# domkirke/acids_transforms

Measured on AMD Instinct MI355X. Metric: spectrogram frames/sec (fwd+invert), n_fft=1024 hop=256, higher is better.
Workload: dtype f32; 1 GPU; configs[1]: batch=1024 clips/GPU x 4 s mono 44.1 kHz, STFT fwd + Magnitude(mel=128, log1p, unipolar) [one fused kernel] + ISTFT invert, fp32; n_fft=1024, hop=256, frames_per_clip=690, clips_per_gpu=1024

## Files before the change

acids_transforms_amd/_lib.py:

```python
import ctypes
import os
import subprocess

import torch

_HERE = os.path.dirname(os.path.abspath(__file__))
_SO = os.environ.get("ACIDS_HIP_LIB") or os.path.join(_HERE, "libacids_hip.so")

ABI_VERSION = 4
AT_OK, AT_EINVAL, AT_EUNSUPPORTED, AT_ENOTINIT, AT_EWORKSPACE, AT_ELAUNCH = 0, -1, -2, -3, -4, -5

c_f = ctypes.c_void_p
c_i64 = ctypes.c_int64
c_int = ctypes.c_int
c_sz = ctypes.c_size_t
c_flt = ctypes.c_float

_SIGNATURES = {
    "at_abi_version": [],
    "at_error_string": [c_int],
    "at_init": [c_int],
    "at_set_variant": [c_int, c_int],
    "at_get_variant": [c_int],
    "at_stft_forward": [c_f, c_i64, c_i64, c_i64, c_i64, c_int, c_int, c_int, c_f, c_f, c_f, c_f],
    "at_stft_mel_forward": [c_f, c_i64, c_i64, c_i64, c_i64, c_int, c_int, c_f, c_f, c_f, c_f, c_int, c_int,
                            c_f, c_int, c_int, c_f, c_f, c_flt, c_f, c_f, c_f, c_int, c_f],
    "at_stft_polar_forward": [c_f, c_i64, c_i64, c_i64, c_i64, c_int, c_int, c_f, c_f, c_f, c_f, c_int, c_int, c_f,
                              c_int, c_f, c_f, c_flt, c_f, c_f, c_f, c_f],
    "at_istft_envelope_table": [c_f, c_int, c_int, c_f, c_f],
    "at_istft_workspace_bytes": [c_i64, c_i64, c_int, c_int],
    "at_istft": [c_f, c_f, c_f, c_i64, c_i64, c_int, c_int, c_f, c_f, c_f, c_f, c_sz, c_f],
    "at_irfft_frames": [c_f, c_f, c_f, c_i64, c_int, c_f, c_f, c_f],
    "at_irfft_frames_streams": [c_f, c_f, c_f, c_i64, c_i64, c_int, c_f, c_f, c_f],
    "at_angle": [c_f, c_i64, c_f, c_f],
    "at_phase_scan": [c_f, c_f, c_i64, c_i64, c_i64, c_int, c_int, c_f, c_f, c_f, c_f, c_f],
    "at_phase_integrate": [c_f, c_i64, c_i64, c_i64, c_int, c_int, c_f, c_f, c_f, c_f],
    "at_polar_to_complex": [c_f, c_f, c_i64, c_f, c_f],
    "at_phase_scan_strided": [c_f, c_f, c_i64, c_i64, c_i64, c_int, c_int, c_f, c_f, c_f, c_f, c_i64, c_f],
    "at_polarif_forward": [c_f, c_i64, c_i64, c_i64, c_int, c_f, c_f, c_f, c_f, c_f, c_f, c_f, c_i64, c_int, c_f, c_f, c_flt,
                           c_f, c_f],
    "at_phase_integrate_polar": [c_f, c_i64, c_i64, c_i64, c_i64, c_int, c_f, c_f, c_f, c_f, c_f],
    "at_cartesian_pack": [c_f, c_i64, c_int, c_f, c_f, c_f, c_f, c_f, c_f],
    "at_cartesian_unpack": [c_f, c_i64, c_int, c_f, c_f, c_f, c_f, c_f, c_f],
    "at_resample_sinc": [c_f, c_i64, c_i64, c_int, c_int, c_int, c_f, c_i64, c_f, c_f],
    "at_sinebank_workspace_bytes": [c_i64, c_int, c_i64, c_int],
    "at_sinebank_offline": [c_f, c_i64, c_i64, c_int, c_f, c_f, c_f, c_i64, c_int, c_f, c_f, c_f, c_f, c_f, c_sz, c_f],
    "at_sinebank_realtime": [c_f, c_i64, c_int, c_int, c_int, c_f, c_f, c_f, c_f, c_f, c_f],
    "at_mel_project": [c_f, c_int, c_i64, c_i64, c_int, c_f, c_int, c_int, c_int, c_int, c_f, c_f, c_flt, c_f, c_i64,
                       c_i64, c_f],
    "at_mel_project_banded": [c_f, c_int, c_i64, c_i64, c_int, c_f, c_f, c_f, c_int, c_int, c_f, c_int, c_int, c_f, c_f,
                              c_flt, c_f, c_i64, c_i64, c_f, c_i64, c_f, c_f, c_f, c_f],
    "at_mel_bf16_bank_bytes": [c_int, c_int],
    "at_mel_bf16_pack_bank": [c_f, c_int, c_int, c_int, c_f, c_f],
    "at_mel_project_bf16": [c_f, c_int, c_i64, c_i64, c_int, c_f, c_int, c_int, c_f, c_f, c_flt, c_f, c_i64, c_f],
    "at_project_small": [c_f, c_i64, c_int, c_f, c_int, c_f, c_f, c_f, c_i64, c_f],
    "at_mag_pointwise": [c_f, c_int, c_i64, c_int, c_int, c_f, c_f, c_flt, c_f, c_f],
    "at_stats_workspace_bytes": [],
    "at_stats": [c_f, c_int, c_i64, c_int, c_flt, c_f, c_f, c_sz, c_f],
    "at_affine": [c_f, c_i64, c_f, c_f, c_int, c_f, c_f],
    "at_pghi_gradients": [c_f, c_i64, c_int, c_int, c_flt, c_int, c_int, c_flt, c_f, c_f, c_f, c_f],
    "at_pghi_offline_workspace_bytes": [c_i64, c_int, c_int],
    "at_pghi_offline": [c_f, c_i64, c_int, c_int, c_flt, c_int, c_int, c_flt, c_flt, c_f, c_f, c_sz, c_f, c_f, c_f],
    "at_pghi_integrate": [c_f, c_f, c_f, c_i64, c_int, c_int, c_flt, c_flt, c_f, c_f, c_sz, c_f, c_f, c_f],
    "at_pghi_rt_workspace_bytes": [c_int, c_int, c_int],
    "at_pghi_realtime": [c_f, c_f, c_f, c_f, c_int, c_int, c_int, c_flt, c_int, c_int, c_flt, c_flt, c_f, c_f, c_f,
                         c_f, c_sz, c_f],
    "at_pghi_realtime_seeded": [c_f, c_f, c_f, c_f, c_int, c_int, c_int, c_flt, c_int, c_int, c_flt, c_flt, c_f, c_f, c_sz,
                                c_f],
    "at_rt_update_buffers": [c_f, c_f, c_int, c_int, c_int, c_f, c_f, c_f, c_f],
    "at_griffinlim_update": [c_f, c_f, c_f, c_flt, c_i64, c_f, c_f],
    "at_istft_griffinlim": [c_f, c_f, c_f, c_flt, c_i64, c_i64, c_int, c_int, c_f, c_f, c_f, c_f],
    "at_scale_complex": [c_f, c_f, c_i64, c_f, c_f],
    "at_oadd_forward": [c_f, c_f, c_int, c_i64, c_int, c_i64, c_f, c_f, c_f],
    "at_oadd_invert": [c_f, c_f, c_int, c_int, c_int, c_int, c_int, c_f, c_f, c_f, c_f],
    "at_oadd_push": [c_f, c_int, c_i64, c_int, c_i64, c_f, c_f],
    "at_mulaw_encode": [c_f, c_i64, c_int, c_f, c_f],
    "at_mulaw_decode": [c_f, c_f, c_i64, c_int, c_f, c_f],
    "at_onehot": [c_f, c_i64, c_int, c_i64, c_f, c_f],
    "at_argmax_last": [c_f, c_f, c_i64, c_int, c_f, c_f],
    "at_stft_backward_workspace_bytes": [c_i64, c_i64, c_int, c_int],
    "at_stft_backward": [c_f, c_i64, c_i64, c_i64, c_int, c_int, c_f, c_f, c_f, c_sz, c_f],
    "at_istft_backward_workspace_bytes": [c_i64, c_i64, c_int, c_int],
    "at_istft_backward": [c_f, c_i64, c_i64, c_int, c_int, c_f, c_f, c_f, c_f, c_f, c_sz, c_f],
    "at_magnitude_backward": [c_f, c_int, c_i64, c_int, c_f, c_int, c_int, c_f, c_f, c_f, c_f, c_int, c_f, c_f, c_f, c_f,
                              c_int, c_int, c_f, c_flt, c_f, c_f, c_f],
    "at_mfcc_backward": [c_f, c_i64, c_i64, c_int, c_f, c_int, c_int, c_int, c_f, c_f, c_f, c_f, c_int, c_f, c_f, c_f, c_f,
                         c_int, c_f, c_f, c_f, c_f],
}
_RESTYPES = {"at_error_string": ctypes.c_char_p, "at_istft_workspace_bytes": c_sz, "at_stats_workspace_bytes": c_sz,
             "at_pghi_offline_workspace_bytes": c_sz, "at_mel_bf16_bank_bytes": c_sz, "at_pghi_rt_workspace_bytes": c_sz,
             "at_sinebank_workspace_bytes": c_sz, "at_stft_backward_workspace_bytes": c_sz,
             "at_istft_backward_workspace_bytes": c_sz}


class AcidsHipError(RuntimeError):
    pass


def build(verbose=False):
    cmd = ["make", "-C", os.path.join(_HERE, "csrc"), "-j4"]
    if not verbose:
        cmd.append("-s")
    subprocess.check_call(cmd)
    return _SO
# ... 110 lines not shown
```

acids_transforms_amd/csrc/capi.hip:

```cpp
#include <hip/hip_runtime.h>
#include <math.h>
#include <stdint.h>
#include <vector>

#include "../../include/acids_hip.h"
#include "autograd.h"
#include "band_bank.h"
#include "fft512.h"

#include <atomic>
#include "variants.h"
namespace at_hip {
int launch_stft1024_fwd(const float*, long long, long long, long long, long long, int, int, const float*,
                        const float2*, float2*, float*, hipStream_t);
int launch_stft1024_h256_fwd(const float*, long long, long long, long long, long long, const float*, const float2*,
                             float2*, float*, const BandBank*, float*, const float*, const float*, float, int, int, int,
                             hipStream_t, const PolarOut* polar = nullptr, int hop = 256);
int launch_istft1024_ola(const float2*, const float*, const float*, long long, long long, int, const float*,
                         const float*, const float2*, float*, hipStream_t, const float2* gl_tprev = nullptr,
                         float gl_mom = 0.f);
int launch_irfft1024_frames(const float2*, const float*, const float*, long long, const float*, const float2*,
                            float*, hipStream_t);
int launch_rfft_generic(const float*, long long, long long, long long, long long, int, int, int, const float*,
                        float2*, float*, hipStream_t);
// ... 15 lines not shown
                         const float*, const float2*, const float2*, float*, hipStream_t);
int launch_stft4096_fwd(const float*, long long, long long, long long, long long, int, int, const float*, const float2*,
                        const float2*, float2*, float*, hipStream_t);
int launch_istft4096_ola(const float2*, const float*, const float*, long long, long long, int, const float*, const float*,
                         const float2*, const float2*, float*, hipStream_t);
int launch_irfft4096_frames(const float2*, const float*, const float*, long long, const float*, const float2*,
                            const float2*, float*, hipStream_t);
int launch_stft_small_fwd(int, const float*, long long, long long, long long, long long, int, int, const float*, const float2*,
                          const float2*, float2*, float*, hipStream_t);
int launch_irfft_small_frames(int, const float2*, const float*, const float*, long long, long long, const float*,
                              const float2*, const float2*, float*, hipStream_t);
int launch_stft512_fwd(const float*, long long, long long, long long, long long, int, int, const float*, const float2*,
                       const float2*, float2*, float*, hipStream_t);
int launch_irfft512_frames(const float2*, const float*, const float*, long long, long long, const float*, const float2*,
                           const float2*, float*, hipStream_t);
int launch_istft512_ola(const float2*, const float*, const float*, long long, long long, int, const float*, const float*,
                        const float2*, const float2*, float*, hipStream_t);

constexpr int kMaxDevices = 16;
static float2* g_twiddles[kMaxDevices] = {nullptr};
static float2* g_tw2048[kMaxDevices] = {nullptr};

static const float2* twiddles_for_current_device() {
  int dev = 0;
  if (hipGetDevice(&dev) != hipSuccess || dev < 0 || dev >= kMaxDevices) return nullptr;
  return g_twiddles[dev];
}

static const float2* tw2048_for_current_device() {
  int dev = 0;
  if (hipGetDevice(&dev) != hipSuccess || dev < 0 || dev >= kMaxDevices) return nullptr;
  return g_tw2048[dev];
}

static bool is_pow2(int n) { return n > 0 && (n & (n - 1)) == 0; }
static bool fft_size_ok(int n) { return n >= 2 && n <= 16384 && (!(n & 1) || n < 8192); }
static bool fft_mixed(int n) { return !is_pow2(n) || n < 8; }

__global__ void envelope_table_kernel(const float* w, int n_fft, int hop, int R, float* env) {
  int i = blockIdx.x * blockDim.x + threadIdx.x;
  if (i >= (1 << R) * hop) return;
  int mask = i / hop, r = i - mask * hop;
  float s = 0.f;
  for (int q = 0; q < R; ++q)
    if (mask & (1 << q)) {
      int o = hop * (R - 1 - q) + r;
      if (o < n_fft) s += w[o] * w[o];
    }
  env[i] = s;
}
static std::atomic<int> g_variants[kVarCount];
int variant(int which) { return g_variants[which].load(std::memory_order_relaxed); }
}

using namespace at_hip;

extern "C" {

int at_abi_version(void) { return 4; }

int at_set_variant(int which, int value) {
  if (which < 0 || which >= kVarCount || value < 0 || value > (which >= kVarFirstPlan ? 65535 : 4)) return AT_EINVAL;
  g_variants[which].store(value, std::memory_order_relaxed);
  return AT_OK;
}

int at_get_variant(int which) {
  if (which < 0 || which >= kVarCount) return AT_EINVAL;
  return g_variants[which].load(std::memory_order_relaxed);
}

const char* at_error_string(int code) {
  switch (code) {
    case AT_OK: return "ok";
    case AT_EINVAL: return "invalid argument";
    case AT_EUNSUPPORTED: return "unsupported configuration";
    case AT_ENOTINIT: return "at_init() not called for this device";
    case AT_EWORKSPACE: return "workspace too small";
    case AT_ELAUNCH: return "HIP launch/runtime error";
    default: return "unknown error";
  }
}

int at_init(int device) {
  if (device < 0 || device >= kMaxDevices) return AT_EINVAL;
  if (g_twiddles[device]) return AT_OK;
  int prev = 0;
  if (hipGetDevice(&prev) != hipSuccess) return AT_ELAUNCH;
  if (hipSetDevice(device) != hipSuccess) return AT_ELAUNCH;
  std::vector<float2> tab(kTwiddleCount);
  const double two_pi = 6.283185307179586476925286766559;
  for (int k = 1; k < 8; ++k)
    for (int l = 0; l < 64; ++l) {
      double a1 = -two_pi * (double)(l * k) / 512.0;
      tab[(k - 1) * 64 + l] = make_float2((float)cos(a1), (float)sin(a1));
      double a2 = -two_pi * (double)((l & 7) * k) / 64.0;
      tab[(7 + k - 1) * 64 + l] = make_float2((float)cos(a2), (float)sin(a2));
    }
  for (int m = 0; m < 8; ++m)
    for (int l = 0; l < 64; ++l) {
      double a = -two_pi * (double)(l + 64 * m) / 1024.0;
      tab[(14 + m) * 64 + l] = make_float2((float)cos(a), (float)sin(a));
    }
  float2* d = nullptr;
  int rc = AT_OK;
  if (hipMalloc((void**)&d, sizeof(float2) * (kTwiddleCount + kTileCtrSlots)) != hipSuccess) rc = AT_ELAUNCH;
  if (rc == AT_OK && hipMemcpy(d, tab.data(), sizeof(float2) * kTwiddleCount, hipMemcpyHostToDevice) != hipSuccess)
    rc = AT_ELAUNCH;
  if (rc == AT_OK && hipMemset(d + kTwiddleCount, 0, sizeof(float2) * kTileCtrSlots) != hipSuccess) rc = AT_ELAUNCH;
  float2* d2 = nullptr;
  if (rc == AT_OK) {
    std::vector<float2> t2(1024 + 256 + 384 + 448 + 2048 + 1536);
    for (int k = 0; k < 2048; ++k) {
      const double a = -two_pi * (double)k / 4096.0;
      t2[2112 + k] = make_float2((float)cos(a), (float)sin(a));
    }
    for (int r = 1; r < 4; ++r)
      for (int k = 0; k < 512; ++k) {
        const double a = -two_pi * (double)(r * k) / 2048.0;
        t2[4160 + (r - 1) * 512 + k] = make_float2((float)cos(a), (float)sin(a));
      }
    for (int r = 1; r < 4; ++r)
      for (int k = 0; k < 128; ++k) {
        const double a = -two_pi * (double)(r * k) / 512.0;
        t2[1280 + (r - 1) * 128 + k] = make_float2((float)cos(a), (float)sin(a));
      }
    for (int r = 1; r < 8; ++r)
      for (int k = 0; k < 64; ++k) {
        const double a = -two_pi * (double)(r * k) / 512.0;
        t2[1664 + (r - 1) * 64 + k] = make_float2((float)cos(a), (float)sin(a));
      }
    for (int k = 0; k < 1024; ++k) {
      const double a = -two_pi * (double)k / 2048.0;
      t2[k] = make_float2((float)cos(a), (float)sin(a));
    }
    for (int k = 0; k < 256; ++k) {
      const double a = -two_pi * (double)k / 512.0;
      t2[1024 + k] = make_float2((float)cos(a), (float)sin(a));
    }
    if (hipMalloc((void**)&d2, sizeof(float2) * t2.size()) != hipSuccess) rc = AT_ELAUNCH;
    if (rc == AT_OK && hipMemcpy(d2, t2.data(), sizeof(float2) * t2.size(), hipMemcpyHostToDevice) != hipSuccess)
      rc = AT_ELAUNCH;
  }
  if (rc == AT_OK) {
    g_tw2048[device] = d2;
    g_twiddles[device] = d;
  }
  (void)hipSetDevice(prev);
  return rc;
}

int at_stft_forward(const float* x, int64_t B, int64_t L, int64_t clip_stride, int64_t T, int n_fft, int hop,
                    int center, const float* window, float* out_complex, float* phase, void* stream) {
  if (B < 0 || T < 0 || L < 0 || hop <= 0 || n_fft <= 0) return AT_EINVAL;
  if (B * T == 0) return AT_OK;
  if (!x || !window || !out_complex) return AT_EINVAL;
  if (!fft_size_ok(n_fft)) return AT_EUNSUPPORTED;
  if (center && L <= n_fft / 2) return AT_EINVAL;
  hipStream_t s = (hipStream_t)stream;
  if (n_fft == 1024 && (((uintptr_t)window) & 7) == 0) {
    const float2* tw = twiddles_for_current_device();
    if (!tw) return AT_ENOTINIT;
    if ((hop == 256 || hop == 128 || hop == 512) && center && (clip_stride & 1) == 0)
      return launch_stft1024_h256_fwd(x, B, L, clip_stride, T, window, tw, (float2*)out_complex, phase, nullptr,
                                      nullptr, nullptr, nullptr, 0.f, 0, 0, 0, s, nullptr, hop);
    return launch_stft1024_fwd(x, B, L, clip_stride, T, hop, center, window, tw, (float2*)out_complex, phase, s);
  }
  if (n_fft == 2048 && (((uintptr_t)window) & 15) == 0) {
    const float2* tw = twiddles_for_current_device();
    const float2* tw2k = tw2048_for_current_device();
    if (!tw || !tw2k) return AT_ENOTINIT;
    return launch_stft2048_fwd(x, B, L, clip_stride, T, hop, center, window, tw, tw2k, (float2*)out_complex, phase, s);
  }
  if (n_fft == 4096 && (((uintptr_t)window) & 15) == 0) {
    const float2* tw = twiddles_for_current_device();
    const float2* tw2k = tw2048_for_current_device();
    if (!tw || !tw2k) return AT_ENOTINIT;
    return launch_stft4096_fwd(x, B, L, clip_stride, T, hop, center, window, tw, tw2k + 2112, (float2*)out_complex, phase, s);
  }
  if ((n_fft == 256 || n_fft == 128) && (((uintptr_t)window) & 7) == 0) {
    const float2* tw = twiddles_for_current_device();
    const float2* tw2k = tw2048_for_current_device();
    if (!tw || !tw2k) return AT_ENOTINIT;
    return launch_stft_small_fwd(n_fft, x, B, L, clip_stride, T, hop, center, window, tw, tw2k + (n_fft == 256 ? 1280 : 1664),
                                 (float2*)out_complex, phase, s);
  }
// ... 381 lines not shown
```

acids_transforms_amd/csrc/fft512.h:

```cpp
#pragma once
#include <hip/hip_runtime.h>

namespace at_hip {

#ifndef AT_WAVE_PRIORITY
#define AT_WAVE_PRIORITY 1
#endif
template <int LEVEL>
__device__ __forceinline__ void wave_priority() {
#if AT_WAVE_PRIORITY
  __builtin_amdgcn_s_setprio(LEVEL);
#endif
}

constexpr int kFftLdsFloat2PerWave = 568;

constexpr int kTwiddleCount = 22 * 64;
constexpr int kTileCtrSlots = 4096;

__device__ __forceinline__ float2 cadd(float2 a, float2 b) { return make_float2(a.x + b.x, a.y + b.y); }

typedef float v2f __attribute__((ext_vector_type(2)));

__device__ __forceinline__ v2f to_v(float2 a) { return (v2f){a.x, a.y}; }
// ... 239 lines not shown
    const v2f a = q[7 - m];
    const v2f b = q[(8 - m) & 7];
    p[m] = (lane == 0) ? b : a;
  }
}

__device__ __forceinline__ void mirror512_rot(const v2f (&v)[8], v2f (&p)[8], int lane, int rot, int col) {
  const int src = (2 * rot - lane) & 63;
  v2f q[8];
#pragma unroll
  for (int m = 0; m < 8; ++m) {
    q[m].x = __shfl(v[m].x, src, 64);
    q[m].y = __shfl(v[m].y, src, 64);
  }
#pragma unroll
  for (int m = 0; m < 8; ++m) {
    const v2f a = q[7 - m];
    const v2f b = q[(8 - m) & 7];
    p[m] = (col == 0) ? b : a;
  }
}

template <typename TW>
__device__ __forceinline__ void rfft_merge(v2f (&v)[8], const TW& tw, int lane, float2& nyq) {
  const v2f hh = {0.5f, 0.5f};
  v2f p[8];
  mirror512(v, p, lane);
  nyq = make_float2(v[0].x - v[0].y, 0.0f);
#pragma unroll
  for (int m = 0; m < 8; ++m) {
    const v2f e = add_conj(v[m], p[m]);
    const v2f d = sub_conj(v[m], p[m]);
    const v2f wd = cmul_v(d, tw.getr(m));
    v[m] = scale_add_mi(e, hh, wd);
  }
}
template <typename TW>
__device__ __forceinline__ void rfft_merge_rot(v2f (&v)[8], const TW& tw, int lane, int rot, int col, float2& nyq) {
  const v2f hh = {0.5f, 0.5f};
  v2f p[8];
  mirror512_rot(v, p, lane, rot, col);
  nyq = make_float2(v[0].x - v[0].y, 0.0f);
#pragma unroll
  for (int m = 0; m < 8; ++m) {
    const v2f e = add_conj(v[m], p[m]);
    const v2f d = sub_conj(v[m], p[m]);
    const v2f wd = cmul_v(d, tw.getr(m));
    v[m] = scale_add_mi(e, hh, wd);
  }
}
template <typename TW>
__device__ __forceinline__ void rfft_merge(float2 (&f)[8], const TW& tw, int lane, float2& nyq) {
  v2f v[8];
#pragma unroll
  for (int m = 0; m < 8; ++m) v[m] = to_v(f[m]);
  rfft_merge(v, tw, lane, nyq);
#pragma unroll
  for (int m = 0; m < 8; ++m) f[m] = to_f2(v[m]);
}

template <typename TW>
__device__ __forceinline__ void irfft_split(v2f (&v)[8], const TW& tw, int lane, float xnyq_re) {
  if (lane == 0) v[0].y = 0.0f;
  v2f p[8];
  mirror512(v, p, lane);
  if (lane == 0) p[0] = (v2f){xnyq_re, 0.0f};
#pragma unroll
  for (int m = 0; m < 8; ++m) {
    const v2f e = add_conj(v[m], p[m]);
    const v2f d = cmul_conj_v(sub_conj(v[m], p[m]), tw.getr(m));
    v[m] = add_pi(e, d);
  }
}
template <typename TW>
__device__ __forceinline__ void irfft_split(float2 (&f)[8], const TW& tw, int lane, float xnyq_re) {
  v2f v[8];
#pragma unroll
  for (int m = 0; m < 8; ++m) v[m] = to_v(f[m]);
  irfft_split(v, tw, lane, xnyq_re);
#pragma unroll
  for (int m = 0; m < 8; ++m) f[m] = to_f2(v[m]);
}

}
```

acids_transforms_amd/csrc/stft1024.hip:

```cpp
#include <hip/hip_runtime.h>
#include "fastmath.h"
#include <type_traits>
#include <stdint.h>
#include <stdlib.h>
#include <stdio.h>
#include <string.h>
#include <atomic>

#include "band_bank.h"
#include "fft512.h"
#include "run_plan.h"
#include "variants.h"

#ifndef AT_ISTFT_NT
#define AT_ISTFT_NT 1
#endif
#ifndef AT_ISTFT_NTLOAD
#define AT_ISTFT_NTLOAD 1
#endif

namespace at_hip {

constexpr int N = 1024;
constexpr int F = 513;
constexpr int WAVES_PER_BLOCK = 4;

struct FwdParams {
  const float* x;
  const float* window;
  const float2* tw;
  float2* out;
  float* phase;
  long long B, L, clip_stride, T;
  long long total_frames;
  long long frames_per_block;
  int hop;
  int center;
};

__device__ __forceinline__ long long reflect_index(long long i, long long L) {
  if (i < 0) i = -i;
  if (i >= L) i = 2 * (L - 1) - i;
  return i;
}

__device__ __forceinline__ void load_frame(const FwdParams& p, long long f, int lane, float2 (&v)[8]) {
  const long long b = f / p.T;
  const long long t = f - b * p.T;
  const float* clip = p.x + b * p.clip_stride;
  const long long start = t * (long long)p.hop - (p.center ? N / 2 : 0);
  const bool interior = (start >= 0) && (start + N <= p.L);
  const bool aligned = (((uintptr_t)(clip + start)) & 7) == 0;
  if (interior && aligned) {
    const float2* src = reinterpret_cast<const float2*>(clip + start);
#pragma unroll
    for (int m = 0; m < 8; ++m) v[m] = src[lane + 64 * m];
  } else if (interior) {
    const float* src = clip + start;
#pragma unroll
    for (int m = 0; m < 8; ++m) {
      v[m].x = src[2 * (lane + 64 * m)];
      v[m].y = src[2 * (lane + 64 * m) + 1];
    }
  } else {
#pragma unroll
    for (int m = 0; m < 8; ++m) {
      long long i0 = start + 2 * (lane + 64 * m);
      if (p.center) {
        v[m].x = clip[reflect_index(i0, p.L)];
        v[m].y = clip[reflect_index(i0 + 1, p.L)];
      } else {
        v[m].x = (i0 < p.L) ? clip[i0] : 0.0f;
        v[m].y = (i0 + 1 < p.L) ? clip[i0 + 1] : 0.0f;
      }
    }
  }
}

template <bool WRITE_PHASE>
__global__ __launch_bounds__(64 * WAVES_PER_BLOCK) void stft1024_fwd_kernel(FwdParams p) {
  __shared__ float2 lds_all[WAVES_PER_BLOCK * kFftLdsFloat2PerWave];
  const int lane = threadIdx.x & 63;
  const int wave = threadIdx.x >> 6;
  float2* lds = lds_all + wave * kFftLdsFloat2PerWave;

  Twiddles tw;
  load_twiddles<false>(tw, p.tw, lane);
  float2 win[8];
#pragma unroll
  for (int m = 0; m < 8; ++m) win[m] = reinterpret_cast<const float2*>(p.window)[lane + 64 * m];

  const long long f_begin = (long long)blockIdx.x * p.frames_per_block;
  long long f_end = f_begin + p.frames_per_block;
  if (f_end > p.total_frames) f_end = p.total_frames;

  long long f = f_begin + wave;
  float2 nxt[8];
  if (f < f_end) load_frame(p, f, lane, nxt);
  for (; f < f_end; f += WAVES_PER_BLOCK) {
    float2 v[8];
#pragma unroll
    for (int m = 0; m < 8; ++m) v[m] = make_float2(nxt[m].x * win[m].x, nxt[m].y * win[m].y);
    if (f + WAVES_PER_BLOCK < f_end) load_frame(p, f + WAVES_PER_BLOCK, lane, nxt);

    fft512<false>(v, tw, lds, lane);
    float2 nyq;
    rfft_merge(v, tw, lane, nyq);

    float2* row = p.out + f * F;
#pragma unroll
    for (int m = 0; m < 8; ++m) row[lane + 64 * m] = v[m];
    if (lane == 0) row[512] = nyq;
    if (WRITE_PHASE) {
      float* prow = p.phase + f * F;
#pragma unroll
      for (int m = 0; m < 8; ++m) prow[lane + 64 * m] = fast_atan2f(v[m].y, v[m].x);
      if (lane == 0) prow[512] = fast_atan2f(nyq.y, nyq.x);
    }
  }
}

struct FwdRunParams {
  const float* x;
  const float* window;
  const float2* tw;
  float2* out;
  float* phase;
  long long B, L, clip_stride, T;
  long long runs_per_clip, frames_per_run;
  BandBank bank;
  float* feat;
  const float* offset;
  const float* scale;
  float eps;
  int contrast;
  int power2;
  int feat_channel_major;
  long long feat_ld, phase_ld;
  const float* ph_offset;
  const float* ph_scale;
  unsigned* tile_ctr;
  unsigned n_tiles;
};

__device__ __forceinline__ float2 load_pair(const float* clip, long long L, long long i0, bool interior, bool aligned,
                                            int lane_off) {
  if (interior) {
    if (aligned) return reinterpret_cast<const float2*>(clip + i0)[lane_off >> 1];
    return make_float2(clip[i0 + lane_off], clip[i0 + lane_off + 1]);
  }
  return make_float2(clip[reflect_index(i0 + lane_off, L)], clip[reflect_index(i0 + lane_off + 1, L)]);
}


__device__ __forceinline__ float fwd_contrast(float v, int mode, float eps) { return band_contrast_fast(v, mode, eps); }

template <bool WRITE_PHASE, int MEL, int FWD_WAVES, bool TWLDS, int CMBUF = 0, bool POLAR = false, int HS = 2, int SP = 0,
          int FQ0 = 0, int FQ1 = 0, bool AL = false, bool NT = false, int HYB = 0, int FC = 1, bool FP2 = false, bool PW = false,
          fqp_t FQP = 0, int FNP = 0>
// ... 107 lines not shown
  if (preloaded) {
#pragma unroll
    for (int m = 0; m < 8; ++m) raw[m] = raw_first[m];
  } else {
    load_first_frame(run, raw);
  }
#pragma unroll
  for (int m = 0; m < 8; ++m) asm volatile("" : "+v"(raw[m].x), "+v"(raw[m].y));
  float2* row = p.out + (b * p.T + t0) * F;
  const long long feat_ld = (POLAR && p.feat_ld) ? p.feat_ld : (long long)p.bank.n_filters;
  const long long phase_ld = (POLAR && p.phase_ld) ? p.phase_ld : F;
  float* prow = (WRITE_PHASE || POLAR) ? p.phase + (b * p.T + t0) * phase_ld : nullptr;
  float* frow = (MEL != 0) ? p.feat + (b * p.T + t0) * feat_ld : nullptr;
  int fc = 0, fhead = 0;
  float* fdst = nullptr;
  if constexpr (FQP != 0) {
    const long long fe0 = (b * p.T + t0) * (long long)F;
    fc = (int)(fe0 & 255);
    fhead = fc;
    fdst = p.feat + (fe0 - fc);
  }
  float ph_off = 0.f, ph_sc = 1.f;
  if (POLAR && p.ph_offset) {
    ph_off = *p.ph_offset;
    ph_sc = *p.ph_scale;
  }
  int rot = 0;
  float2* sp = nullptr;
  v2f carry = {0.f, 0.f};
  bool head = true;
  if constexpr (AL) {
    static_assert(MEL != 2 && !WRITE_PHASE && !POLAR && TWLDS, "aligned stream stores: spectrum out, LDS twiddles");
    const long long e0 = (b * p.T + t0) * F;
    rot = (int)(e0 & 63);
    sp = p.out + (e0 - rot) + lane;
  }
  auto put = [&](float2* dst, v2f val) {
    if (NT) __builtin_nontemporal_store(val, reinterpret_cast<v2f*>(dst));
    else *reinterpret_cast<v2f*>(dst) = val;
  };
  long long t_cur = t0;
  float cm[CMBUF ? CMBUF : 1][8];
  int cm_held[CMBUF ? CMBUF : 1];
#pragma unroll
  for (int q = 0; q < (CMBUF ? CMBUF : 1); ++q) {
    cm_held[q] = 0;
#pragma unroll
    for (int k = 0; k < 8; ++k) cm[q][k] = 0.f;
  }
  float mel_off = 0.f, mel_inv = 1.f;
  if (MEL != 0 && p.offset) {
    mel_off = *p.offset;
    mel_inv = 1.0f / *p.scale;
  }

  float2 nyq_pending = make_float2(0.f, 0.f);
  float2* nyq_dst = nullptr;
  auto flush_nyquist = [&]() {
    if (nyq_dst != nullptr && lane == 0) *nyq_dst = nyq_pending;
    if (WRITE_PHASE && nyq_dst != nullptr && lane == 0)
      p.phase[(nyq_dst - p.out)] = fast_atan2f(nyq_pending.y, nyq_pending.x);
  };
  auto frame_body = [&](const float2 (&fresh)[HS]) {
    wave_priority<3>();
    float2 v[8];
#pragma unroll
    for (int m = 0; m < 8; ++m) {
      const v2f w = (HYB & 2) ? win_regs[m] : lds_read_single(reinterpret_cast<const v2f*>(win) + lane + 64 * m);
      v[m] = make_float2(raw[m].x * w.x, raw[m].y * w.y);
    }
#pragma unroll
    for (int m = 0; m < 8 - HS; ++m) raw[m] = raw[m + HS];
#pragma unroll
    for (int k = 0; k < HS; ++k) raw[8 - HS + k] = fresh[k];
    float2 nyq;
    const int col = AL ? ((lane - rot) & 63) : lane;
    {
      v2f z[8];
#pragma unroll
      for (int m = 0; m < 8; ++m) z[m] = to_v(v[m]);
      if constexpr (AL && (HYB & 1)) {
        fft512<false>(z, tw_hyb, lds, lane, col);
        tw_hyb.col = col;
        rfft_merge_rot(z, tw_hyb, lane, rot, col, nyq);
      } else if constexpr (AL) {
        fft512<false>(z, tw_lds, lds, lane, col);
        const LdsTwiddles<false> tw_col = {tab, col};
        rfft_merge_rot(z, tw_col, lane, rot, col, nyq);
      } else if constexpr (TWLDS && (HYB & 1)) {
        fft512<false>(z, tw_hyb, lds, lane);
        rfft_merge(z, tw_hyb, lane, nyq);
      } else if (TWLDS) {
        fft512<false>(z, tw_lds, lds, lane);
        rfft_merge(z, tw_lds, lane, nyq);
      } else {
        fft512<false>(z, tw_regs, lds, lane);
        rfft_merge(z, tw_regs, lane, nyq);
      }
#pragma unroll
      for (int m = 0; m < 8; ++m) v[m] = to_f2(z[m]);
      if constexpr (AL) {
        wave_priority<1>();
        const bool lo = lane < rot;
        const v2f s0 = lo ? carry : z[0];
        if (head) {
          if (!lo) put(sp, s0);
          head = false;
        } else {
          put(sp, s0);
        }
#pragma unroll
        for (int j = 1; j < 8; ++j) put(sp + 64 * j, lo ? z[j - 1] : z[j]);
        carry = lo ? z[7] : (v2f){nyq.x, 0.f};
        if (rot == 63) {
          put(sp + 512, carry);
          sp += 576;
          rot = 0;
        } else {
          sp += 512;
          ++rot;
        }
      }
    }
    if (MEL != 2 && !AL) {
#pragma unroll
      for (int m = 0; m < 8; ++m) row[lane + 64 * m] = v[m];
    }
    if (WRITE_PHASE) {
#pragma unroll
      for (int m = 0; m < 8; ++m) prow[lane + 64 * m] = fast_atan2f(v[m].y, v[m].x);
      prow += F;
    }
    if (POLAR) {
#pragma unroll
      for (int m = 0; m < 8; ++m) {
        float ph = fast_atan2f(v[m].y, v[m].x);
        if (p.ph_offset) ph = (ph - ph_off) / ph_sc;
        prow[lane + 64 * m] = ph;
      }
      if (lane == 0) {
        float ph = fast_atan2f(nyq.y, nyq.x);
        if (p.ph_offset) ph = (ph - ph_off) / ph_sc;
        prow[512] = ph;
      }
      prow += phase_ld;
    }
    auto cm_push = [&](auto cmsel, int f, float value) {
      constexpr int CMROW = decltype(cmsel)::value;
      if (f >= 0) {
#pragma unroll
        for (int k = 0; k < 7; ++k) cm[CMROW][k] = cm[CMROW][k + 1];
        cm[CMROW][7] = value;
      }
      ++cm_held[CMROW];
      if (f >= 0) {
        const long long e = ((long long)b * p.bank.n_filters + f) * p.T + t_cur + 1;
        if ((e & 7) == 0 || t_cur == t1 - 1) {
          float* dst = p.feat + e - 8;
          if (cm_held[CMROW] >= 8) {
            if ((e & 3) == 0) {
              reinterpret_cast<float4*>(dst)[0] = make_float4(cm[CMROW][0], cm[CMROW][1], cm[CMROW][2], cm[CMROW][3]);
              reinterpret_cast<float4*>(dst)[1] = make_float4(cm[CMROW][4], cm[CMROW][5], cm[CMROW][6], cm[CMROW][7]);
            } else {
#pragma unroll
              for (int k = 0; k < 8; ++k) dst[k] = cm[CMROW][k];
            }
          } else {
#pragma unroll
            for (int k = 0; k < 8; ++k)
              if (k >= 8 - cm_held[CMROW]) dst[k] = cm[CMROW][k];
          }
          cm_held[CMROW] = 0;
        }
      }
    };
    wave_priority<0>();
    if constexpr (MEL != 0 && FQ0 > 0) {
      static_assert(SP == 2 && (CMBUF == 0 || CMBUF == 2) && !POLAR, "fixed-length epilogue: two passes, no phase rows");
      float* absrow = reinterpret_cast<float*>(lds);
      wave_lds_sync();
// ... 183 lines not shown
    if (lane < rot) put(sp, carry);
  }
  if constexpr (FQP != 0) {
    wave_lds_sync();
    const float* fbuf = reinterpret_cast<const float*>(lds) - 2 * kFeatCarry;
    const float4 v = reinterpret_cast<const float4*>(fbuf)[lane];
    const float vv[4] = {v.x, v.y, v.z, v.w};
#pragma unroll
    for (int c = 0; c < 4; ++c)
      if (4 * lane + c < fc && 4 * lane + c >= fhead) fdst[4 * lane + c] = vv[c];
    wave_lds_sync();
  }
  };

  if constexpr (!PW) {
    do_run((long long)blockIdx.x * FWD_WAVES + wave, true);
  } else {
    for (int it = 0;; ++it) {
      const unsigned tile = __builtin_amdgcn_readfirstlane(s_tile[it & 1]);
      if (tile >= p.n_tiles) break;
      unsigned nxt = 0;
      if (threadIdx.x == 0) nxt = atomicAdd(p.tile_ctr, 1u);
      do_run((long long)tile * FWD_WAVES + wave, false);
      if (threadIdx.x == 0) s_tile[(it + 1) & 1] = nxt;
      __syncthreads();
    }
    if (threadIdx.x == 0) {
      if (atomicAdd(p.tile_ctr + 1, 1u) == gridDim.x - 1) {
        atomicExch(p.tile_ctr, 0u);
        atomicExch(p.tile_ctr + 1, 0u);
      }
    }
  }
}

enum { IN_COMPLEX = 0, IN_POLAR = 1, IN_GL = 2 };
enum { OUT_OLA = 0, OUT_FRAMES = 1 };

struct InvParams {
  const float2* X;
  const float* mag;
  const float* phase;
  const float2* tprev;
  float gl_mom;
  const float* window;
  const float* env;
  const float2* tw;
  float* y;
  long long B, T;
  long long runs_per_clip;
  long long slots_per_run;
  long long total_frames, frames_per_block;
};

__device__ __forceinline__ void sincos_big(float phase, float& s, float& c) {
  double t = (double)phase * 0.15915494309189533577;
  t -= rint(t);
  const float r = (float)t;
  s = __builtin_amdgcn_sinf(r);
  c = __builtin_amdgcn_cosf(r);
}

typedef float f32x2 __attribute__((ext_vector_type(2)));
template <int IN_MODE>
struct RawFrame;
template <>
struct RawFrame<IN_COMPLEX> {
  f32x2 d[8];
  float ny0;
};
template <>
struct RawFrame<IN_POLAR> {
  float a[8], ph[8];
  float ny0, ny1;
};
template <>
struct RawFrame<IN_GL> {
  f32x2 r[8], t[8];
  float a[8];
  f32x2 rny, tny;
  float any;
};

__device__ __forceinline__ void load_raw(const InvParams& p, long long f, int lane, RawFrame<IN_COMPLEX>& q) {
  const f32x2* row = reinterpret_cast<const f32x2*>(p.X + f * F);
#pragma unroll
  for (int m = 0; m < 8; ++m) {
#if AT_ISTFT_NTLOAD
    q.d[m] = __builtin_nontemporal_load(row + lane + 64 * m);
#else
    q.d[m] = row[lane + 64 * m];
#endif
  }
  q.ny0 = reinterpret_cast<const float*>(row + 512)[0];
}
__device__ __forceinline__ void load_raw(const InvParams& p, long long f, int lane, RawFrame<IN_POLAR>& q) {
  const float* mrow = p.mag + f * F;
  const float* prow = p.phase + f * F;
#pragma unroll
  for (int m = 0; m < 8; ++m) {
    q.a[m] = mrow[lane + 64 * m];
    q.ph[m] = prow[lane + 64 * m];
  }
  q.ny0 = mrow[512];
  q.ny1 = prow[512];
}

__device__ __forceinline__ void load_raw(const InvParams& p, long long f, int lane, RawFrame<IN_GL>& q) {
  const f32x2* rrow = reinterpret_cast<const f32x2*>(p.X + f * F);
  const f32x2* trow = reinterpret_cast<const f32x2*>(p.tprev + f * F);
  const float* mrow = p.mag + f * F;
#pragma unroll
  for (int m = 0; m < 8; ++m) {
    q.r[m] = rrow[lane + 64 * m];
    q.t[m] = trow[lane + 64 * m];
    q.a[m] = mrow[lane + 64 * m];
  }
  q.rny = rrow[512];
  q.tny = trow[512];
  q.any = mrow[512];
}

__device__ __forceinline__ float2 gl_update(f32x2 r, f32x2 t, float mag, float mom) {
  float ax = r.x, ay = r.y;
  ax -= mom * t.x;
  ay -= mom * t.y;
  const float d = __builtin_amdgcn_sqrtf(fmaf(ax, ax, ay * ay)) + 1e-16f;
  const float s = mag * __builtin_amdgcn_rcpf(d);
  return make_float2(s * ax, s * ay);
}

__device__ __forceinline__ void raw_to_spectrum(const RawFrame<IN_COMPLEX>& q, float2 (&v)[8], float& nyq_re) {
#pragma unroll
  for (int m = 0; m < 8; ++m) v[m] = make_float2(q.d[m].x, q.d[m].y);
  nyq_re = q.ny0;
}
__device__ __forceinline__ void raw_to_spectrum(const RawFrame<IN_POLAR>& q, float2 (&v)[8], float& nyq_re) {
#pragma unroll
  for (int m = 0; m < 8; ++m) {
    float sn, cs;
    sincos_big(q.ph[m], sn, cs);
    v[m] = make_float2(q.a[m] * cs, q.a[m] * sn);
  }
  float sn, cs;
  sincos_big(q.ny1, sn, cs);
  nyq_re = q.ny0 * cs;
}

__device__ __forceinline__ void raw_to_spectrum(const RawFrame<IN_GL>& q, float2 (&v)[8], float& nyq_re, float mom) {
#pragma unroll
  for (int m = 0; m < 8; ++m) v[m] = gl_update(q.r[m], q.t[m], q.a[m], mom);
  nyq_re = gl_update(q.rny, q.tny, q.any, mom).x;
}

template <int IN_MODE>
__device__ __forceinline__ void load_spectrum(const InvParams& p, long long f, int lane, float2 (&v)[8], float& nyq_re) {
  RawFrame<IN_MODE> q;
  load_raw(p, f, lane, q);
  raw_to_spectrum(q, v, nyq_re);
}

__device__ __forceinline__ float2 scaled_window(const float* window, int i) {
  const float2 w = reinterpret_cast<const float2*>(window)[i];
  return make_float2(w.x * (1.0f / 1024.0f), w.y * (1.0f / 1024.0f));
}

template <typename TW>
__device__ __forceinline__ void synth_frame_nowin(const float2 (&v)[8], float nyq_re, const TW& tw, float2* lds, int lane,
                                                  v2f (&z)[8]) {
#pragma unroll
  for (int m = 0; m < 8; ++m) z[m] = to_v(v[m]);
  irfft_split(z, tw, lane, nyq_re);
  fft512<true>(z, tw, lds, lane);
}
__device__ __forceinline__ v2f ola_window(const float2* win, int lane, int m) {
  return lds_read_single(reinterpret_cast<const v2f*>(win) + lane + 64 * m);
}

template <typename TW>
__device__ __forceinline__ void synth_frame(float2 (&v)[8], float nyq_re, const TW& tw, const float2* win,
                                            float2* lds, int lane) {
  v2f z[8];
#pragma unroll
  for (int m = 0; m < 8; ++m) z[m] = to_v(v[m]);
  irfft_split(z, tw, lane, nyq_re);
  fft512<true>(z, tw, lds, lane);
#pragma unroll
  for (int m = 0; m < 8; ++m) {
    const v2f w = lds_read_single(reinterpret_cast<const v2f*>(win) + lane + 64 * m);
    v[m] = to_f2(z[m] * w);
  }
}

template <int IN_MODE, int DEPTH, bool TWLDS, int HS = 2>
__global__ __launch_bounds__(64 * WAVES_PER_BLOCK, IN_MODE == IN_GL ? 2 : (TWLDS ? 5 : 4) - DEPTH) void istft1024_ola_kernel(InvParams p) {
  constexpr int R = 8 / HS;
  constexpr int C = 4 / HS;
  constexpr int H = 128 * HS;
  constexpr int kFull = (1 << R) - 1;
  __shared__ float2 lds_all[WAVES_PER_BLOCK * kFftLdsFloat2PerWave + 512 + (TWLDS ? kTwiddleCount : 0)];
  const int lane = threadIdx.x & 63;
  const int wave = __builtin_amdgcn_readfirstlane(threadIdx.x >> 6);
  float2* lds = lds_all + wave * kFftLdsFloat2PerWave;
  float2* win = lds_all + WAVES_PER_BLOCK * kFftLdsFloat2PerWave;
  float2* twtab = win + 512;
  for (int i = threadIdx.x; i < 512; i += 64 * WAVES_PER_BLOCK) win[i] = scaled_window(p.window, i);
  if (TWLDS)
    for (int i = threadIdx.x; i < kTwiddleCount; i += 64 * WAVES_PER_BLOCK) twtab[i] = p.tw[i];
  __syncthreads();

  const long long run = (long long)blockIdx.x * WAVES_PER_BLOCK + wave;
  const long long b = run / p.runs_per_clip;
  if (b >= p.B) return;
  const long long r = run - b * p.runs_per_clip;
  const long long nslots = p.T - 1;
  const long long j0 = r * p.slots_per_run;
  long long j1 = j0 + p.slots_per_run;
  if (j1 > nslots) j1 = nslots;
  if (j0 >= j1) return;

  Twiddles tw_regs;
  if (!TWLDS) load_twiddles<true>(tw_regs, p.tw, lane);
  const LdsTwiddles<true> tw_lds = {twtab, lane};
  auto synth = [&](const float2 (&v)[8], float nyq, v2f (&z)[8]) {
    if (TWLDS) synth_frame_nowin(v, nyq, tw_lds, lds, lane, z);
    else synth_frame_nowin(v, nyq, tw_regs, lds, lane, z);
  };

  v2f acc[8];
#pragma unroll
  for (int m = 0; m < 8; ++m) acc[m] = (v2f){0.f, 0.f};

  const long long fbase = b * p.T;
  float* yclip = p.y + b * (H * nslots);
  long long t = (j0 + C - (R - 1) > 0) ? j0 + C - (R - 1) : 0;
  const long long t_last = j1 - 1 + C;
  const long long t_have = (t_last < p.T - 1) ? t_last : p.T - 1;

  RawFrame<IN_MODE> q0 = {}, q1 = {};
  if (t <= t_have) load_raw(p, fbase + t, lane, q0);
  if (t + 1 <= t_have) load_raw(p, fbase + t + 1, lane, q1);

  auto consume = [&](const RawFrame<IN_MODE>& q) {
    float2 v[8];
    float nyq;
    if constexpr (IN_MODE == IN_GL) raw_to_spectrum(q, v, nyq, p.gl_mom);
    else raw_to_spectrum(q, v, nyq);
    v2f z[8];
    synth(v, nyq, z);
#pragma unroll
    for (int m = 0; m < 8; ++m) acc[m] = __builtin_elementwise_fma(z[m], ola_window(win, lane, m), acc[m]);
  };
  auto put_y = [&](float2* dst, float2 val) {
#if AT_ISTFT_NT
    __builtin_nontemporal_store((v2f){val.x, val.y}, reinterpret_cast<v2f*>(dst));
#else
    *dst = val;
#endif
  };
  static_assert(sizeof(v2f) == sizeof(float2), "");
  auto emit = [&](long long j, const float2* env) {
    float2* dst = reinterpret_cast<float2*>(yclip + j * H);
#pragma unroll
    for (int k = 0; k < HS; ++k) {
      const float2 e = env[lane + 64 * k];
      put_y(dst + lane + 64 * k, make_float2(acc[k].x / e.x, acc[k].y / e.y));
    }
  };
// ... 545 lines not shown
```

include/acids_hip.h:

```cpp
#ifndef ACIDS_HIP_H
#define ACIDS_HIP_H

#include <stddef.h>
#include <stdint.h>

#ifdef __cplusplus
extern "C" {
#endif

#define AT_OK 0
#define AT_EINVAL (-1)
#define AT_EUNSUPPORTED (-2)
#define AT_ENOTINIT (-3)
#define AT_EWORKSPACE (-4)
#define AT_ELAUNCH (-5)

int at_abi_version(void);
const char *at_error_string(int code);

#define AT_VARIANT_EPILOGUE 0
#define AT_VARIANT_FRAME_KERNELS 1
#define AT_VARIANT_SMALL_PROJECTION 2
#define AT_VARIANT_SCAN_LAYOUT 3
#define AT_VARIANT_PGHI_KERNEL 4
#define AT_VARIANT_ISTFT_RUNS 5
#define AT_VARIANT_RUN_LENGTH 6
#define AT_VARIANT_ISTFT_TILE 7
#define AT_VARIANT_ROW_RUN 8
int at_set_variant(int which, int value);
int at_get_variant(int which);

int at_init(int device);

int at_stft_forward(const float *x, int64_t B, int64_t L, int64_t clip_stride, int64_t T, int n_fft, int hop,
                    int center, const float *window, float *out_complex, float *phase, void *stream);

int at_stft_mel_forward(const float *x, int64_t B, int64_t L, int64_t clip_stride, int64_t T, int n_fft, int hop,
                        const float *window, const int32_t *lane_filter, const int32_t *lane_start,
                        const float *band_weights, int n_filters, int n_passes, const int32_t *pass_len_host,
                        int contrast, int power2, const float *offset, const float *scale, float eps,
                        float *out_complex_or_null, float *phase_or_null, float *feat, int feat_channel_major,
                        void *stream);

int at_stft_polar_forward(const float *x, int64_t B, int64_t L, int64_t clip_stride, int64_t T, int n_fft, int hop,
                          const float *window, const int32_t *lane_filter, const int32_t *lane_start,
                          const float *band_weights, int n_filters, int n_passes, const int32_t *pass_len_host,
                          int contrast, const float *mag_offset, const float *mag_scale, float eps,
                          const float *phase_offset, const float *phase_scale, float *out_stacked, void *stream);

int at_istft_envelope_table(const float *inv_window, int n_fft, int hop, float *env16, void *stream);

size_t at_istft_workspace_bytes(int64_t B, int64_t T, int n_fft, int hop);

int at_istft(const float *X_complex, const float *mag, const float *phase, int64_t B, int64_t T, int n_fft, int hop,
             const float *inv_window, const float *env16, float *y, void *workspace, size_t workspace_bytes,
             void *stream);

int at_irfft_frames(const float *X_complex, const float *mag, const float *phase, int64_t nframes, int n_fft,
                    const float *inv_window, float *frames, void *stream);

int at_irfft_frames_streams(const float *X_complex, const float *mag, const float *phase, int64_t nframes,
                            int64_t frames_per_stream, int n_fft, const float *inv_window, float *frames,
                            void *stream);

int at_mel_project(const void *A, int a_kind, int64_t rows, int64_t lda, int K, const float *bank, int ldb, int N,
                   int contrast, int inverse, const float *offset, const float *scale, float eps, float *out,
                   int64_t ld_out, int64_t T_transposed, void *stream);

size_t at_mel_bf16_bank_bytes(int K, int N);
int at_mel_bf16_pack_bank(const float *bank, int K, int ldb, int N, void *bank_bf16, void *stream);
int at_mel_project_bf16(const void *A, int a_kind, int64_t rows, int64_t lda, int K, const void *bank_bf16, int N,
                        int contrast, const float *offset, const float *scale, float eps, float *out, int64_t ld_out,
                        void *stream);

int at_mag_pointwise(const void *A, int a_kind, int64_t n, int contrast, int inverse, const float *offset,
                     const float *scale, float eps, float *out, void *stream);

size_t at_stats_workspace_bytes(void);
int at_stats(const void *A, int a_kind, int64_t n, int contrast, float eps, double *out4, void *workspace,
             size_t workspace_bytes, void *stream);

int at_affine(const float *x, int64_t n, const float *offset, const float *scale, int inverse, float *out,
              void *stream);

int at_pghi_gradients(const float *mag, int64_t B, int T, int F, float gamma, int n_fft, int hop, float eps,
                      float *tgradw, float *fgradw, float *spec_or_null, void *stream);

size_t at_pghi_offline_workspace_bytes(int64_t B, int T, int F);

int at_pghi_offline(const float *mag, int64_t B, int T, int F, float gamma, int n_fft, int hop, float tol,
                    float abstol, float *phase, void *workspace, size_t workspace_bytes, int64_t *npops_or_null,
                    int32_t *order_or_null, void *stream);

int at_pghi_integrate(const float *mag, const float *tgradw, const float *fgradw, int64_t B, int T, int F, float tol,
                      float abstol, float *phase, void *workspace, size_t workspace_bytes, int64_t *npops_or_null,
                      int32_t *order_or_null, void *stream);

size_t at_pghi_rt_workspace_bytes(int S, int n, int F);

int at_pghi_realtime(const float *mag_hist, const float *mag, const float *prev_phase, const float *noise, int S,
                     int n, int F, float gamma, int n_fft, int hop, float tol, float eps, float *phase,
                     float *tgradw_or_null, float *fgradw_or_null, void *workspace, size_t workspace_bytes,
                     void *stream);

int at_pghi_realtime_seeded(const float *mag_hist, const float *mag, const float *prev_phase, uint32_t *rng_state, int S,
                            int n, int F, float gamma, int n_fft, int hop, float tol, float eps, float *phase,
                            void *workspace, size_t workspace_bytes, void *stream);

int at_rt_update_buffers(const float *mag, const float *phase, int S, int n, int F, const float *hist_in,
                         float *hist_out, float *phase_out, void *stream);

int at_angle(const float *x_complex, int64_t n, float *out, void *stream);

int at_cartesian_pack(const float *x_complex, int64_t rows, int F, const float *re_offset, const float *re_scale,
                      const float *im_offset, const float *im_scale, float *stacked, void *stream);
// ... 86 lines not shown
```

Before: 448.8 million frames/s.

## Load mirrored bins per lane so the inverse real-FFT split pairs bins locally

The inverse STFT loader now has odd-indexed register slots fetch the mirrored bin (64-lane)&63 instead of lane+64m. Each lane then holds both partners of a conjugate-symmetric pair, and the real-FFT split runs with local arithmetic plus four cross-lane shuffles for the odd outputs. An optional paired forward merge is added but stays off unless AT_MIRROR_LOCAL>=2. A host-side twiddle table export is also added. The aim is to cut the cross-lane shuffle and permute cost of the irfft split, at the price of scattered global loads and extra selects for lane 0.

```diff
diff --git a/acids_transforms_amd/_lib.py b/acids_transforms_amd/_lib.py
--- a/acids_transforms_amd/_lib.py
+++ b/acids_transforms_amd/_lib.py
@@ -20,6 +20,7 @@
     "at_abi_version": [],
     "at_error_string": [c_int],
     "at_init": [c_int],
+    "at_twiddle_table": [c_f, c_int],
     "at_set_variant": [c_int, c_int],
     "at_get_variant": [c_int],
     "at_stft_forward": [c_f, c_i64, c_i64, c_i64, c_i64, c_int, c_int, c_int, c_f, c_f, c_f, c_f],
diff --git a/acids_transforms_amd/csrc/capi.hip b/acids_transforms_amd/csrc/capi.hip
--- a/acids_transforms_amd/csrc/capi.hip
+++ b/acids_transforms_amd/csrc/capi.hip
@@ -121,13 +121,7 @@
   }
 }
 
-int at_init(int device) {
-  if (device < 0 || device >= kMaxDevices) return AT_EINVAL;
-  if (g_twiddles[device]) return AT_OK;
-  int prev = 0;
-  if (hipGetDevice(&prev) != hipSuccess) return AT_ELAUNCH;
-  if (hipSetDevice(device) != hipSuccess) return AT_ELAUNCH;
-  std::vector<float2> tab(kTwiddleCount);
+static void fill_twiddle_table(float2* tab) {
   const double two_pi = 6.283185307179586476925286766559;
   for (int k = 1; k < 8; ++k)
     for (int l = 0; l < 64; ++l) {
@@ -141,6 +135,23 @@
       double a = -two_pi * (double)(l + 64 * m) / 1024.0;
       tab[(14 + m) * 64 + l] = make_float2((float)cos(a), (float)sin(a));
     }
+}
+
+int at_twiddle_table(float* table_host, int count) {
+  if (table_host == nullptr || count != kTwiddleCount) return AT_EINVAL;
+  fill_twiddle_table(reinterpret_cast<float2*>(table_host));
+  return AT_OK;
+}
+
+int at_init(int device) {
+  if (device < 0 || device >= kMaxDevices) return AT_EINVAL;
+  if (g_twiddles[device]) return AT_OK;
+  int prev = 0;
+  if (hipGetDevice(&prev) != hipSuccess) return AT_ELAUNCH;
+  if (hipSetDevice(device) != hipSuccess) return AT_ELAUNCH;
+  std::vector<float2> tab(kTwiddleCount);
+  fill_twiddle_table(tab.data());
+  const double two_pi = 6.283185307179586476925286766559;
   float2* d = nullptr;
   int rc = AT_OK;
   if (hipMalloc((void**)&d, sizeof(float2) * (kTwiddleCount + kTileCtrSlots)) != hipSuccess) rc = AT_ELAUNCH;
diff --git a/acids_transforms_amd/csrc/fft512.h b/acids_transforms_amd/csrc/fft512.h
--- a/acids_transforms_amd/csrc/fft512.h
+++ b/acids_transforms_amd/csrc/fft512.h
@@ -345,4 +345,97 @@
   for (int m = 0; m < 8; ++m) f[m] = to_f2(v[m]);
 }
 
-}
+#ifndef AT_MIRROR_LOCAL
+#define AT_MIRROR_LOCAL 1
+#endif
+
+__device__ __forceinline__ int paired_bin(int lane) { return (64 - lane) & 63; }
+
+__device__ __forceinline__ v2f conj_add_pi(v2f e, v2f d) {
+  v2f r;
+  asm("v_pk_add_f32 %0, %1, %2 op_sel:[0,1] op_sel_hi:[1,0] neg_hi:[1,0]" : "=v"(r) : "v"(e), "v"(d));
+  return r;
+}
+
+__device__ __forceinline__ v2f getr_by_lane(const Twiddles& tw, int m_rest, int m_lane0, int lane) {
+  return lane == 0 ? tw.tr[m_lane0] : tw.tr[m_rest];
+}
+template <bool INV>
+__device__ __forceinline__ v2f getr_by_lane(const LdsTwiddles<INV>& tw, int m_rest, int m_lane0, int lane) {
+  return tw.getr(lane == 0 ? m_lane0 : m_rest);
+}
+__device__ __forceinline__ v2f getr_by_lane(const HybridTwiddles& tw, int m_rest, int m_lane0, int lane) {
+  return tw.getr(lane == 0 ? m_lane0 : m_rest);
+}
+
+template <typename TW>
+__device__ __forceinline__ void irfft_split_paired(v2f (&v)[8], const TW& tw, int lane, float xnyq_re) {
+  const bool z0 = lane == 0;
+  auto pair = [](v2f a, v2f b, v2f w, v2f& z, v2f& zp) {
+    const v2f e = add_conj(a, b);
+    const v2f d = cmul_conj_v(sub_conj(a, b), w);
+    z = add_pi(e, d);
+    zp = conj_add_pi(e, d);
+  };
+  const v2f a0 = {v[0].x, z0 ? 0.0f : v[0].y};
+  const v2f b0 = z0 ? (v2f){xnyq_re, 0.0f} : v[7];
+  v2f z[5], zp[5];
+  pair(a0, b0, tw.getr(0), z[0], zp[0]);
+  pair(z0 ? v[3] : v[2], v[5], getr_by_lane(tw, 2, 3, lane), z[1], zp[1]);
+  pair(v[4], z0 ? v[4] : v[3], tw.getr(4), z[2], zp[2]);
+  pair(z0 ? v[7] : v[6], v[1], getr_by_lane(tw, 6, 7, lane), z[3], zp[3]);
+  pair(v[2], v[6], tw.getr(2), z[4], zp[4]);
+  v[0] = z[0];
+  v[2] = z0 ? z[4] : z[1];
+  v[4] = z[2];
+  v[6] = z0 ? zp[4] : z[3];
+  const v2f o1 = zp[3];
+  const v2f o3 = z0 ? z[1] : zp[2];
+  const v2f o5 = zp[1];
+  const v2f o7 = z0 ? z[3] : zp[0];
+  const int src = paired_bin(lane);
+  v[1] = (v2f){__shfl(o1.x, src, 64), __shfl(o1.y, src, 64)};
+  v[3] = (v2f){__shfl(o3.x, src, 64), __shfl(o3.y, src, 64)};
+  v[5] = (v2f){__shfl(o5.x, src, 64), __shfl(o5.y, src, 64)};
+  v[7] = (v2f){__shfl(o7.x, src, 64), __shfl(o7.y, src, 64)};
+}
+
+__device__ __forceinline__ v2f conj_scale_add_mi(v2f e, v2f hh, v2f wd) {
+  v2f r;
+  asm("v_pk_fma_f32 %0, %1, %2, %3 op_sel:[0,0,1] op_sel_hi:[1,1,0] neg_lo:[0,0,1] neg_hi:[1,0,1]" : "=v"(r) : "v"(e), "s"(hh), "v"(wd));
+  return r;
+}
+template <typename TW>
+__device__ __forceinline__ void rfft_merge_paired(v2f (&v)[8], const TW& tw, int src, int col, float2& nyq) {
+  const v2f hh = {0.5f, 0.5f};
+  const bool z0 = col == 0;
+  nyq = make_float2(v[0].x - v[0].y, 0.0f);
+  auto swap_odd = [&](v2f (&u)[8]) {
+#pragma unroll
+    for (int m = 1; m < 8; m += 2) u[m] = (v2f){__shfl(u[m].x, src, 64), __shfl(u[m].y, src, 64)};
+  };
+  auto pair = [&](v2f a, v2f b, v2f w, v2f& x, v2f& xp) {
+    const v2f e = add_conj(a, b);
+    const v2f wd = cmul_v(sub_conj(a, b), w);
+    x = scale_add_mi(e, hh, wd);
+    xp = conj_scale_add_mi(e, hh, wd);
+  };
+  swap_odd(v);
+  v2f x[5], xp[5];
+  pair(v[0], z0 ? v[0] : v[7], tw.getr(0), x[0], xp[0]);
+  pair(z0 ? v[3] : v[2], v[5], getr_by_lane(tw, 2, 3, col), x[1], xp[1]);
+  pair(v[4], z0 ? v[4] : v[3], tw.getr(4), x[2], xp[2]);
+  pair(z0 ? v[7] : v[6], v[1], getr_by_lane(tw, 6, 7, col), x[3], xp[3]);
+  pair(v[2], v[6], tw.getr(2), x[4], xp[4]);
+  v[0] = x[0];
+  v[2] = z0 ? x[4] : x[1];
+  v[4] = x[2];
+  v[6] = z0 ? xp[4] : x[3];
+  v[1] = xp[3];
+  v[3] = z0 ? x[1] : xp[2];
+  v[5] = xp[1];
+  v[7] = z0 ? x[3] : xp[0];
+  swap_odd(v);
+}
+
+}
diff --git a/acids_transforms_amd/csrc/stft1024.hip b/acids_transforms_amd/csrc/stft1024.hip
--- a/acids_transforms_amd/csrc/stft1024.hip
+++ b/acids_transforms_amd/csrc/stft1024.hip
@@ -75,6 +75,23 @@
       }
     }
   }
+}
+
+template <typename TW>
+__device__ __forceinline__ void merge_spectrum(v2f (&z)[8], const TW& tw, int lane, float2& nyq) {
+#if AT_MIRROR_LOCAL >= 2
+  rfft_merge_paired(z, tw, paired_bin(lane), lane, nyq);
+#else
+  rfft_merge(z, tw, lane, nyq);
+#endif
+}
+template <typename TW>
+__device__ __forceinline__ void merge_spectrum_rot(v2f (&z)[8], const TW& tw, int lane, int rot, int col, float2& nyq) {
+#if AT_MIRROR_LOCAL >= 2
+  rfft_merge_paired(z, tw, (2 * rot - lane) & 63, col, nyq);
+#else
+  rfft_merge_rot(z, tw, lane, rot, col, nyq);
+#endif
 }
 
 template <bool WRITE_PHASE>
@@ -348,20 +365,20 @@
       if constexpr (AL && (HYB & 1)) {
         fft512<false>(z, tw_hyb, lds, lane, col);
         tw_hyb.col = col;
-        rfft_merge_rot(z, tw_hyb, lane, rot, col, nyq);
+        merge_spectrum_rot(z, tw_hyb, lane, rot, col, nyq);
       } else if constexpr (AL) {
         fft512<false>(z, tw_lds, lds, lane, col);
         const LdsTwiddles<false> tw_col = {tab, col};
-        rfft_merge_rot(z, tw_col, lane, rot, col, nyq);
+        merge_spectrum_rot(z, tw_col, lane, rot, col, nyq);
       } else if constexpr (TWLDS && (HYB & 1)) {
         fft512<false>(z, tw_hyb, lds, lane);
-        rfft_merge(z, tw_hyb, lane, nyq);
+        merge_spectrum(z, tw_hyb, lane, nyq);
       } else if (TWLDS) {
         fft512<false>(z, tw_lds, lds, lane);
-        rfft_merge(z, tw_lds, lane, nyq);
+        merge_spectrum(z, tw_lds, lane, nyq);
       } else {
         fft512<false>(z, tw_regs, lds, lane);
-        rfft_merge(z, tw_regs, lane, nyq);
+        merge_spectrum(z, tw_regs, lane, nyq);
       }
 #pragma unroll
       for (int m = 0; m < 8; ++m) v[m] = to_f2(z[m]);
@@ -711,14 +728,30 @@
   float any;
 };
 
+__device__ __forceinline__ int raw_bin(int lane, int m) {
+#if AT_MIRROR_LOCAL
+  return ((m & 1) ? paired_bin(lane) : lane) + 64 * m;
+#else
+  return lane + 64 * m;
+#endif
+}
+template <typename TW>
+__device__ __forceinline__ void split_spectrum(v2f (&z)[8], const TW& tw, int lane, float nyq_re) {
+#if AT_MIRROR_LOCAL
+  irfft_split_paired(z, tw, lane, nyq_re);
+#else
+  irfft_split(z, tw, lane, nyq_re);
+#endif
+}
+
 __device__ __forceinline__ void load_raw(const InvParams& p, long long f, int lane, RawFrame<IN_COMPLEX>& q) {
   const f32x2* row = reinterpret_cast<const f32x2*>(p.X + f * F);
 #pragma unroll
   for (int m = 0; m < 8; ++m) {
 #if AT_ISTFT_NTLOAD
-    q.d[m] = __builtin_nontemporal_load(row + lane + 64 * m);
+    q.d[m] = __builtin_nontemporal_load(row + raw_bin(lane, m));
 #else
-    q.d[m] = row[lane + 64 * m];
+    q.d[m] = row[raw_bin(lane, m)];
 #endif
   }
   q.ny0 = reinterpret_cast<const float*>(row + 512)[0];
@@ -728,8 +761,8 @@
   const float* prow = p.phase + f * F;
 #pragma unroll
   for (int m = 0; m < 8; ++m) {
-    q.a[m] = mrow[lane + 64 * m];
-    q.ph[m] = prow[lane + 64 * m];
+    q.a[m] = mrow[raw_bin(lane, m)];
+    q.ph[m] = prow[raw_bin(lane, m)];
   }
   q.ny0 = mrow[512];
   q.ny1 = prow[512];
@@ -741,9 +774,9 @@
   const float* mrow = p.mag + f * F;
 #pragma unroll
   for (int m = 0; m < 8; ++m) {
-    q.r[m] = rrow[lane + 64 * m];
-    q.t[m] = trow[lane + 64 * m];
-    q.a[m] = mrow[lane + 64 * m];
+    q.r[m] = rrow[raw_bin(lane, m)];
+    q.t[m] = trow[raw_bin(lane, m)];
+    q.a[m] = mrow[raw_bin(lane, m)];
   }
   q.rny = rrow[512];
   q.tny = trow[512];
@@ -799,7 +832,7 @@
                                                   v2f (&z)[8]) {
 #pragma unroll
   for (int m = 0; m < 8; ++m) z[m] = to_v(v[m]);
-  irfft_split(z, tw, lane, nyq_re);
+  split_spectrum(z, tw, lane, nyq_re);
   fft512<true>(z, tw, lds, lane);
 }
 __device__ __forceinline__ v2f ola_window(const float2* win, int lane, int m) {
@@ -812,7 +845,7 @@
   v2f z[8];
 #pragma unroll
   for (int m = 0; m < 8; ++m) z[m] = to_v(v[m]);
-  irfft_split(z, tw, lane, nyq_re);
+  split_spectrum(z, tw, lane, nyq_re);
   fft512<true>(z, tw, lds, lane);
 #pragma unroll
   for (int m = 0; m < 8; ++m) {
diff --git a/include/acids_hip.h b/include/acids_hip.h
--- a/include/acids_hip.h
+++ b/include/acids_hip.h
@@ -31,6 +31,7 @@
 int at_get_variant(int which);
 
 int at_init(int device);
+int at_twiddle_table(float *table_host, int count);
 
 int at_stft_forward(const float *x, int64_t B, int64_t L, int64_t clip_stride, int64_t T, int n_fft, int hop,
                     int center, const float *window, float *out_complex, float *phase, void *stream);
```

Result: no change. 452.4 million frames/s (median of 3 runs) (+0.8%).
